# exoclime/HELIOS

Hardware: AMD Instinct MI355X
Metric: rad-conv iterations/sec x (lambda-bins x layers) (higher is better)
Workload: dtype f64; 1 GPU; BASELINE config 2: single column, 10 000 bins x 100 layers, premixed corr-k, isotropic scattering; nbin=10000, nlayer=100, ny=20, species=0, columns_per_gpu=1, columns_total=1, loop=radiative, parallelism=columns sharded, 1 per GPU

## Files before the change

### helios_amd/csrc/rt_coef_kernel.inc

```
template <int ROWS, int COEF_TPB>
__global__ void __launch_bounds__(64 * COEF_TPB) HX_COEF_KERNEL(KArgs a HX_PLANE_ARG) {
    using CT = HX_PLANE_T;
    extern __shared__ __align__(16) double smem[];
    const int col = blockIdx.y;
    if (a.done[col]) return;
    const int wave = threadIdx.x >> 6, lane = threadIdx.x & 63;
    const int ntiles = a.nblk_x * a.nparts * a.NW;
    const int TS = COEF_TPB * a.S;
    const int TSP = TS;
    const int NBX = a.coef_nbx;
    double* sh_lay = smem;
    double* sh_int = sh_lay + (size_t)a.L * TSP;
    double* sh_ray = sh_int + (size_t)a.I * TSP;
    double* sh_mu = sh_ray + (size_t)a.H * NBX;
    double* sh_dc = sh_mu + a.H;
    const size_t ncl = a.cloud_lds ? (size_t)a.H * NBX : 0;
    double* sh_g0 = sh_dc + a.H;
    double* sh_cab = sh_g0 + ncl;
    double* sh_csc = sh_cab + ncl;
    int* c_of_q = (int*)(sh_csc + ncl);
    int* x_of_q = c_of_q + TS;
    const size_t nc = (size_t)a.Y * a.X;
    const size_t wgI = nc * a.I;
    const int x_base = (blockIdx.x * COEF_TPB) / (a.NW * a.nparts) * a.nxb;
    for (int q = threadIdx.x; q < TS; q += blockDim.x) {
        const int tl = blockIdx.x * COEF_TPB + q / a.S, s_in_wave = q % a.S;
        int c = -1, xq = x_base;
        if (tl < ntiles) {
            const int wv = tl % a.NW, part = (tl / a.NW) % a.nparts, bx = tl / (a.NW * a.nparts);
            const int s_local = wv * a.S + s_in_wave;
            const int xl = s_local / a.ypb, yl = s_local - xl * a.ypb;
            const int x = bx * a.nxb + xl, y = part * a.ypb + yl;
            if (s_local < a.G && x < a.X) { c = y + a.Y * x; xq = x; }
        }
        c_of_q[q] = c;
        x_of_q[q] = xq;
    }
    {
        const double* mml = a.mmm_lay + (size_t)col * a.I;
        const double* mmi = a.mmm_int + (size_t)col * a.I;
        const double* dcu = a.dcol_u + (size_t)col * a.L;
        const double* dcl = a.dcol_l + (size_t)col * a.L;
        const double* pint = a.p_int + (size_t)col * a.I;
        const double grav = a.colpar[col].g;
        for (int h = threadIdx.x; h < a.H; h += blockDim.x) {
            if (a.iso) {
                sh_mu[h] = mml[h];
                sh_dc[h] = (pint[h] - pint[h + 1]) / grav;
            } else {
                const int i = h >> 1, ii = i + (h & 1);
                sh_mu[h] = (mmi[ii] + mml[i]) / 2.0;
                sh_dc[h] = (h & 1) ? dcu[i] : dcl[i];
            }
        }
        for (int t = threadIdx.x; t < a.H * NBX; t += blockDim.x) {
            const int xs = t / a.H, h = t - xs * a.H, x = min(x_base + xs, a.X - 1);
            const size_t src = ((size_t)col * a.X + x) * a.H + h;
            sh_ray[(size_t)h * NBX + xs] = a.half_ray[src];
            if (a.cloud_lds) {
                sh_g0[(size_t)h * NBX + xs] = a.half_g0[src];
                sh_cab[(size_t)h * NBX + xs] = a.half_cab[src];
                sh_csc[(size_t)h * NBX + xs] = a.half_csc[src];
            }
        }
    }
    __syncthreads();
    {
        const int q0 = threadIdx.x % TS, nrun = blockDim.x / TS, run = threadIdx.x / TS;
        const int cq = c_of_q[q0];
        if (a.from_table) {
            const size_t sp = nc, st = nc * a.npress;
            const double* ktable = a.coltab[col].k;
            for (int pass = 0; pass < (a.iso ? 1 : 2); pass++) {
                const int nlev = pass == 0 ? a.L : a.I;
                const TPIndex* tp = (pass == 0 ? a.tp_lay : a.tp_int) + (size_t)col * a.I;
                double* dst = pass == 0 ? sh_lay : sh_int;
                const int per = (nlev + nrun - 1) / nrun;
                const int l0 = run * per, l1 = min(nlev, l0 + per);
                int ktd = -1, ktu = -1, kpd = -1, kpu = -1;
                double c00 = 0, c01 = 0, c10 = 0, c11 = 0;
                TPIndex knext = tp[min(l0, nlev - 1)];
                for (int lev = l0; lev < l1; lev++) {
                    double v = 0.0;
                    const TPIndex k = knext;
                    knext = tp[min(lev + 1, nlev - 1)];
                    if (cq >= 0) {
                        if (k.tdown != ktd || k.tup != ktu || k.pdown != kpd || k.pup != kpu) {
                            const double* t0 = ktable + (size_t)cq + st * k.tdown;
                            const double* t1 = ktable + (size_t)cq + st * k.tup;
                            c00 = t0[sp * k.pdown];
                            c01 = t0[sp * k.pup];
                            c10 = t1[sp * k.pdown];
                            c11 = t1[sp * k.pup];
                            ktd = k.tdown; ktu = k.tup; kpd = k.pdown; kpu = k.pup;
                        }
                        v = blend_tp(c00, c01, c10, c11, k, false);
                    }
                    dst[(size_t)lev * TSP + q0] = v;
                }
            }
        } else {
            const double* opl = a.opac_wg_lay + col * wgI;
            const double* opi = a.opac_wg_int + col * wgI;
            for (int lev = run; lev < a.L; lev += nrun)
                sh_lay[(size_t)lev * TSP + q0] = cq >= 0 ? opl[(size_t)cq + nc * lev] : 0.0;
            if (!a.iso)
                for (int lev = run; lev < a.I; lev += nrun)
                    sh_int[(size_t)lev * TSP + q0] = cq >= 0 ? opi[(size_t)cq + nc * lev] : 0.0;
        }
    }
    __syncthreads();
    const int tl = blockIdx.x * COEF_TPB + wave;
    if (tl >= ntiles) return;
    const int j = lane % a.k, q = wave * a.S + lane / a.k;
    const int c = c_of_q[q], x = x_of_q[q], xs = x - x_base;
    const bool valid = c >= 0;
    const hx_rt_column cp = a.colpar[col];
    CT* ctile = HX_PLANES + col * a.coef_col + (size_t)tl * a.nplane * ROWS * 64;
    const double nmu = -cp.mu_star;
    const bool plain = a.clouds != 1 && a.scat_corr != 1 && a.g_0 == 0.0 && a.dir_beam != 1;
    const double* Fd = a.F_dir_wg + col * wgI;
    const double* Fc = a.Fc_dir_wg + col * wgI;
    auto beam_at_node = [&](int n) -> double {
        if (!(a.dir_beam == 1 && valid && n <= a.H)) return 0.0;
        if (a.iso) return Fd[(size_t)c + nc * n];
        return (n & 1) ? Fc[(size_t)c + nc * (n >> 1)] : Fd[(size_t)c + nc * (n >> 1)];
    };
    double F_here = beam_at_node(j * ROWS), F_above = beam_at_node(j * ROWS + 1);
    bool scatters = true;
    if (a.matrix) {
        bool mine = false;
#pragma unroll 1
        for (int r = 0; r < ROWS; r++) {
            const int h = j * ROWS + r;
            if (valid && h < a.H) {
                const int i = a.iso ? h : h >> 1;
                const bool lower = a.iso || (h & 1) == 0;
                const int ii = lower ? i : i + 1;
                double ray = 0.0, csc = 0.0, cab = 0.0;
                if (a.cloud_lds) {
                    cab = sh_cab[(size_t)h * NBX + xs];
                    csc = sh_csc[(size_t)h * NBX + xs];
                } else if (a.clouds == 1) {
                    const size_t src = ((size_t)col * a.X + x) * a.H + h;
                    cab = a.half_cab[src];
                    csc = a.half_csc[src];
                }
                if (a.scat == 1) ray = sh_ray[(size_t)h * NBX + xs];
                const double o_l = sh_lay[(size_t)i * TSP + q], o_i = a.iso ? o_l : sh_int[(size_t)ii * TSP + q];
                const double kap = a.iso ? o_l : (lower ? (o_i + o_l) / 2.0 : (o_l + o_i) / 2.0);
                mine = mine || single_scat_albedo(ray + csc, kap * sh_mu[h] + cab, a.w_0_limit) > a.w_0_scat_limit;
            }
        }
        const unsigned long long votes = __ballot(mine);
        const unsigned long long group = a.k >= 64 ? ~0ull : ((1ull << a.k) - 1ull) << (lane - j);
        scatters = (votes & group) != 0ull;
        if (valid && j == 0) a.trigger[col * nc + c] = scatters ? 1 : 0;
    }
    for (int r = 0; r < ROWS; r++) {
        const int h = j * ROWS + r;
        double alpha = 1.0, beta = 0.0, up = 0.0, vp = 0.0, dd = 0.0, du = 0.0;
        const double Fbot = F_here, Ftop = F_above;
        F_here = F_above;
        F_above = beam_at_node(h + 2);
        if (valid && h < a.H) {
            const int i = a.iso ? h : h >> 1;
            const bool lower = a.iso || (h & 1) == 0;
            const int ii = lower ? i : i + 1;
            double g0 = a.g_0, ray = 0.0, csc = 0.0, cab = 0.0;
            if (a.cloud_lds) {
                g0 = sh_g0[(size_t)h * NBX + xs];
                cab = sh_cab[(size_t)h * NBX + xs];
                csc = sh_csc[(size_t)h * NBX + xs];
            } else if (a.clouds == 1) {
                const size_t src = ((size_t)col * a.X + x) * a.H + h;
                g0 = a.half_g0[src];
                cab = a.half_cab[src];
                csc = a.half_csc[src];
            }
            if (a.scat == 1) ray = sh_ray[(size_t)h * NBX + xs];
            const double o_l = sh_lay[(size_t)i * TSP + q], o_i = a.iso ? o_l : sh_int[(size_t)ii * TSP + q];
            const double kap = a.iso ? o_l : (lower ? (o_i + o_l) / 2.0 : (o_l + o_i) / 2.0);
            const double mu = sh_mu[h], dcol = sh_dc[h];
            const double w0 = single_scat_albedo(ray + csc, kap * mu + cab, a.w_0_limit);
            const double dtau_gas = dcol * (kap + ray / mu);
            const double dtau = plain ? dtau_gas : dtau_gas + dcol * (cab + csc) / mu;
            const Slab s = plain ? slab_coeffs_plain(w0, dtau, a.epsi)
                                 : slab_coeffs(w0, dtau, g0, a.epsi, a.epsi2, cp.mu_star, a.scat_corr, a.i2s, a.dir_beam == 1);
            if (a.diag != nullptr && a.dir_beam == 1) {
                if (s.nlim) atomicAdd(a.diag + HX_DIAG_G_LIMITED, (unsigned long long)s.nlim);
            }
            double invM = 1.0 / s.M;
            alpha = s.P * invM;
            beta = -s.N * invM;
            double K = 2.0 * HX_PI * a.epsi * (1.0 - w0) / (s.E - w0);
            double u, v;
            if (!scatters) {
                alpha = s.trans;
                beta = 0.0;
                invM = 1.0;
                K = 2.0 * HX_PI * a.epsi;
                if (a.iso || dtau < a.dtau_limit) {
                    u = v = (1.0 - s.trans) / 2.0;
                } else {
                    const double gq = a.epsi * (s.trans - 1.0) / dtau;
                    u = 1.0 + gq;
                    v = -s.trans - gq;
                }
            } else if (a.iso || dtau < a.dtau_limit) {
                u = v = (s.N + s.M - s.P) / 2.0;
            } else {
                const double qq = (plain ? a.epsi : a.epsi / (s.E * (1.0 - w0 * g0))) * (s.P - s.M + s.N) / dtau;
                u = (s.M + s.N) + qq;
                v = -s.P - qq;
            }
            up = K * u * invM;
            vp = K * v * invM;
            if (a.dir_beam == 1 && scatters) {
                const double dn = Fbot / nmu * (s.Gm * s.M + s.Gp * s.N) - Ftop / nmu * s.Gm * s.P;
                const double upw = Ftop / nmu * (s.Gm * s.N + s.Gp * s.M) - Fbot / nmu * s.P * s.Gp;
                dd = dmin(0.0, dn) * invM;
                du = dmin(0.0, upw) * invM;
            }
            if (h == 0) {
                a.boaK[col * nc + c] = scatters ? (1.0 - w0) / (s.E - w0) : 1.0;
                a.Fdir0[col * nc + c] = a.dir_beam == 1 ? (a.F_dir_wg + col * wgI)[c] : 0.0;
            }
        }
        const size_t off = plane_off(r, lane, ROWS);
        if constexpr (sizeof(CT) == sizeof(double)) {
            __builtin_nontemporal_store(alpha, ctile + 0 * ROWS * 64 + off);
            __builtin_nontemporal_store(beta, ctile + 1 * ROWS * 64 + off);
            __builtin_nontemporal_store(up, ctile + 2 * ROWS * 64 + off);
            if (a.has_vp) __builtin_nontemporal_store(vp, ctile + (size_t)a.pl_vp * ROWS * 64 + off);
        } else {
            __builtin_nontemporal_store(plane0_code(alpha, beta), ctile + 0 * ROWS * 64 + off);
            __builtin_nontemporal_store(plane1_code(beta), ctile + 1 * ROWS * 64 + off);
            __builtin_nontemporal_store((CT)up, ctile + 2 * ROWS * 64 + off);
            if (a.has_vp) __builtin_nontemporal_store((CT)(up + vp), ctile + (size_t)a.pl_vp * ROWS * 64 + off);
        }
        if (a.dir_beam == 1) {
            __builtin_nontemporal_store((CT)dd, ctile + (size_t)a.pl_dd * ROWS * 64 + off);
            __builtin_nontemporal_store((CT)du, ctile + (size_t)(a.pl_dd + 1) * ROWS * 64 + off);
        }
    }
}
```

### helios_amd/csrc/rt_fused.h

```cpp
#pragma once
#include <string>
#include <vector>

#include "hx_common.h"

namespace hx {

struct TileGeom {
    int k, ROWS, S;
    int nxb, ypb, nparts, G, NW, threads;
    int nblk_x;
    int nblk;
    int nplane;
    int has_vp, pl_vp, pl_dd;
    size_t tile_rows;
    size_t coef_elems_per_col, flux_elems_per_col;
};

struct Species {
    double* pretab = nullptr;
    double* scat_cross = nullptr;
    double* vmr_tab = nullptr;
    bool vmr_from_tab = false;
    double weight = 0.0;
// ... 9 lines not shown
    const double *lam, *scat, *absorb;
    int nw, nr;
};

struct ProfileEntry {
    std::string name;
    hipEvent_t e0, e1;
};

}

struct hx_rt {
    hx_context* ctx;
    hx_rt_dims d;
    hx_rt_flags f;
    std::vector<hx_rt_column> cols;
    int X, Y, L, I, H, C, nsweep;
    hx::TileGeom g;
    bool have_grid = false, have_tables = false, have_planck = false, refreshed = false;
    bool keep_down = false;
    bool opac_stale = false;
    void* tp_lay = nullptr;
    void* tp_int = nullptr;
    double *T_lay_ref = nullptr, *T_int_ref = nullptr;
    int nchunk;
    int coef_tpb = 4;
    bool cloud_lds = true;
    bool serpentine = false;
    unsigned flux_launches = 0;
    double state_cache_mb = 0;
    bool generic_scans = false;
    bool conv_shmem_raised = false;
    bool coef_shmem_raised = false;

    double *interwave = nullptr, *deltawave = nullptr, *wave = nullptr, *gauss_y = nullptr,
           *gauss_w = nullptr, *ktemp = nullptr, *kpress = nullptr;
    std::vector<hx::TableSet> tables;
    std::vector<int> col_table;
    hx::TableSet* coltab = nullptr;
    hx::TableSet* coltab_ref = nullptr;
    double* planck_grid = nullptr;
    std::vector<hx::Species> species;
    void* species_dev = nullptr;
    int* abs_list = nullptr;
    int nabs = 0;
    bool species_dev_stale = true;
    double *fac_lay = nullptr, *fac_int = nullptr;
    double *spec_lay = nullptr, *spec_int = nullptr;
    double *sc_spec_lay = nullptr, *sc_spec_int = nullptr;

    hx_rt_column* colpar = nullptr;
    double *p_lay = nullptr, *p_int = nullptr, *dcol_u = nullptr, *dcol_l = nullptr;
    double *T_lay = nullptr, *T_int = nullptr;
    double *surf_albedo = nullptr, *starflux = nullptr, *Bstar = nullptr;
    double *opac_wg_lay = nullptr, *opac_wg_int = nullptr;
    double *scat_cross_lay = nullptr, *scat_cross_int = nullptr;
    double *mmm_lay = nullptr, *mmm_int = nullptr;
    double *cl_abs_lay = nullptr, *cl_abs_int = nullptr, *cl_sc_lay = nullptr, *cl_sc_int = nullptr,
           *cl_g0_lay = nullptr, *cl_g0_int = nullptr, *g0_tot_lay = nullptr, *g0_tot_int = nullptr;
    double *half_ray = nullptr, *half_g0 = nullptr, *half_cab = nullptr, *half_csc = nullptr;
    double *vmr_lay = nullptr, *vmr_int = nullptr;
    double *delta_z = nullptr, *z_lay = nullptr;
    double *dtau_u = nullptr, *dtau_l = nullptr;
    double *F_dir_wg = nullptr, *Fc_dir_wg = nullptr;
    double* F_dir_band_n = nullptr;
    double* Bn = nullptr;
// ... 49 lines not shown
```

### helios_amd/csrc/rt_fused.hip

```cpp
#include "hx_tool.h"
#include "rt_select.h"
#include "rt_species.h"

#include <algorithm>
#include <cmath>

using namespace hx;

namespace {

int rt_fail(hx_rt* rt, int code, const char* msg) { return hx_fail(rt->ctx, code, "%s", msg); }

template <class T>
int dev_alloc(hx_rt* rt, T** p, size_t n, bool zero = true) {
    void* q = nullptr;
    if (n == 0) n = 1;
    hipError_t e = hipMalloc(&q, n * sizeof(T));
    if (e != hipSuccess)
        return hx_fail(rt->ctx, -(int)e, "hipMalloc of %zu bytes failed: %s", n * sizeof(T),
                       hipGetErrorString(e));
    if (zero) {
        e = hipMemsetAsync(q, 0, n * sizeof(T), rt->ctx->stream);
        if (e != hipSuccess) return hx_fail(rt->ctx, -(int)e, "hipMemset failed");
    }
// ... 180 lines not shown
    f.keep_up = rt->matrix_keep_state ? 1 : 0;
    f.colpar = a.colpar;
    f.Bn = a.Bn; f.coef = a.coef; f.U0_in = a.U0; f.boaK = a.boaK; f.Fdir0 = a.Fdir0;
    f.surf_albedo = a.surf_albedo; f.gauss_w = a.gauss_w;
    f.Utile = a.Utile; f.Dtile = a.Dtile; f.U0 = a.U0; f.F_down_band_n = a.F_down_band_n;
    f.F_up_band_n = a.F_up_band_n;
    f.coef_col = a.coef_col; f.flux_col = a.flux_col;
    f.done = a.done;
    f.reverse = rt->serpentine ? (rt->flux_launches++ & 1) : 0;
    f.cache_state_from = INT_MAX;
    if (rt->serpentine && rt->state_cache_mb > 0) {
        const double per_wg = (double)g.nparts * g.NW * g.ROWS * 64 * sizeof(double);
        const long long total = (long long)g.nblk_x * rt->C;
        const long long keep = (long long)(rt->state_cache_mb * 1048576.0 / per_wg);
        f.cache_state_from = (int)std::max(0LL, total - keep);
    }
    if (rt->matrix) {
        f.reverse = 0;
        f.cache_state_from = INT_MAX;
    }
    (void)(rt->coef32 ? select_flux_f32(rt, &f) : select_flux<double>(rt, &f));
}

void launch_coef(hx_rt* rt, KArgs a) {
    const TileGeom& g = rt->g;
    const int ntiles = g.nblk_x * g.nparts * g.NW, tpb = rt->coef_tpb;
    a.coef_nbx = coef_nbx(rt, tpb);
    size_t shmem = coef_shmem_bytes(rt, tpb);
    const size_t cloud_image = 3 * (size_t)rt->H * a.coef_nbx * sizeof(double);
    a.cloud_lds = a.clouds == 1 && rt->cloud_lds && shmem + cloud_image <= 80 * 1024;
    if (a.cloud_lds) shmem += cloud_image;
    const dim3 grid((ntiles + tpb - 1) / tpb, rt->C);
    if (rt->coef32) select_coef_f32(rt, a, grid, shmem);
    else select_coef<double>(rt, a, grid, shmem);
}

int set_flux_shmem_limits(hx_rt* rt) {
    const size_t shmem = flux_shmem_bytes(rt);
    if (shmem > 160 * 1024) return rt_fail(rt, HX_E_UNSUPPORTED, "workgroup LDS demand exceeds 160 KiB");
    if (shmem <= 64 * 1024) return 0;
    HX_HIP(rt->ctx, rt->coef_bytes == 4 ? select_flux_f32(rt, nullptr) : select_flux<double>(rt, nullptr));
    return 0;
}

}

extern "C" {

int hx_rt_struct_sizes(int* dims_size, int* flags_size, int* column_size) {
    if (dims_size) *dims_size = (int)sizeof(hx_rt_dims);
    if (flags_size) *flags_size = (int)sizeof(hx_rt_flags);
    if (column_size) *column_size = (int)sizeof(hx_rt_column);
    return 0;
}

static int rt_create_into(hx_rt* rt, hx_context* ctx, const hx_rt_dims* dims, const hx_rt_flags* flags,
                          const hx_rt_column* columns);

int hx_rt_create(hx_context* ctx, const hx_rt_dims* dims, const hx_rt_flags* flags,
                 const hx_rt_column* columns, hx_rt** out_rt) {
    if (!ctx || !dims || !flags || !columns || !out_rt) return HX_E_ARG;
    *out_rt = nullptr;
    HX_REQUIRE(ctx, dims->nbin > 0 && dims->ny > 0 && dims->nlayer >= 1 && dims->ncol > 0, HX_E_ARG,
               "bad dimensions");
    HX_REQUIRE(ctx, dims->plancktable_dim >= 10 && dims->plancktable_step > 0, HX_E_ARG,
               "bad Planck-table dimensions");
    HX_HIP(ctx, hipSetDevice(ctx->device));
// ... 9 lines not shown

static int rt_create_into(hx_rt* rt, hx_context* ctx, const hx_rt_dims* dims, const hx_rt_flags* flags,
                          const hx_rt_column* columns) {
    rt->ctx = ctx;
    rt->d = *dims;
    rt->f = *flags;
    rt->cols.assign(columns, columns + dims->ncol);
    rt->X = dims->nbin; rt->Y = dims->ny; rt->L = dims->nlayer; rt->I = rt->L + 1;
    rt->H = flags->iso ? rt->L : 2 * rt->L;
    rt->C = dims->ncol;
    rt->have_albedo.assign(dims->ncol, 0);
    rt->col_table.assign(dims->ncol, 0);
    RT_ALLOC(rt->iter_dev, 2);
    rt->nsweep = (flags->singlewalk ? 1000 : 3) * (flags->scat ? 1 : 0) + 1;
#ifdef HX_PROFILING
    if (const char* e = getenv("HELIOS_RT_DEBUG_NSWEEP")) rt->nsweep = atoi(e);
#endif
    if (const char* e = getenv("HELIOS_RT_MATRIX"))
        return hx_fail(ctx, HX_E_ARG, "HELIOS_RT_MATRIX=%s: the knob is retired (the matrix method has one solver); unset it", e);
    rt->matrix = flags->matrix != 0;
    rt->matrix_keep_state = rt->matrix && flags->debug == 1;
    if (!choose_geometry(rt->H, rt->Y, rt->X, rt->C, flags->dir_beam, flags->scat_corr, rt->g))
        return hx_fail(ctx, HX_E_UNSUPPORTED, "fused path supports nlayer <= 1024 (2048 isothermal layers); use the per-stage API");
    rt->nchunk = std::max(1, std::min(512, std::max((rt->X + 47) / 48, std::min(32, (rt->X + 7) / 8))));
    if (const char* e = getenv("HELIOS_RT_GENERIC_SCANS")) rt->generic_scans = atoi(e) != 0;
    rt->coef_bytes = flags->coef_fp32 && !rt->matrix && coef_fp32_tiling(rt->g.ROWS, rt->g.k, rt->generic_scans) ? 4 : 8;
    if (const char* e = getenv("HELIOS_RT_CLOUD_LDS")) rt->cloud_lds = atoi(e) != 0;
    rt->coef_tpb = std::max(1, std::min(8, 16 / std::max(1, rt->g.S)));
    if (const char* e = getenv("HELIOS_RT_COEF_TPB")) rt->coef_tpb = atoi(e);
    if (rt->coef_tpb != 1 && rt->coef_tpb != 2 && !(rt->coef_tpb == 8 && rt->g.ROWS <= 16)) rt->coef_tpb = 4;
    while (rt->coef_tpb > 1 && coef_shmem_bytes(rt, rt->coef_tpb) > 150 * 1024) rt->coef_tpb /= 2;
    if (coef_shmem_bytes(rt, rt->coef_tpb) > 160 * 1024)
        return hx_fail(ctx, HX_E_UNSUPPORTED, "k_rt_coef's staging of one tile exceeds the 160 KiB of LDS");
    if (const char* e = getenv("HELIOS_RT_NCHUNK")) rt->nchunk = std::max(1, std::min(4096, atoi(e)));
    {
        const double state_mb = (double)rt->C * rt->g.flux_elems_per_col * sizeof(double) / 1048576.0;
        const double between_mb = (double)rt->C * rt->X * ((rt->H + 3) + 4.0 * rt->I) * sizeof(double) / 1048576.0;
        rt->serpentine = state_mb >= 64.0 && between_mb <= 64.0;
        rt->state_cache_mb = rt->serpentine ? 240.0 : 0.0;
    }
    if (const char* e = getenv("HELIOS_RT_SERPENTINE")) rt->serpentine = atoi(e) != 0;
    if (const char* e = getenv("HELIOS_RT_STATE_CACHE_MB")) rt->state_cache_mb = atof(e);
    rt->species.resize(dims->nspecies > 0 ? dims->nspecies : 0);
    int rc = set_flux_shmem_limits(rt);
    if (rc) return rc;

    const size_t X = rt->X, Y = rt->Y, L = rt->L, I = rt->I, C = rt->C, nc = X * Y;
    RT_ALLOC(rt->interwave, X + 1); RT_ALLOC(rt->deltawave, X); RT_ALLOC(rt->wave, X);
    RT_ALLOC(rt->gauss_y, Y); RT_ALLOC(rt->gauss_w, Y);
    RT_ALLOC(rt->ktemp, dims->ntemp); RT_ALLOC(rt->kpress, dims->npress);
    RT_ALLOC(rt->planck_grid, (size_t)(dims->plancktable_dim + 1) * X);
    RT_ALLOC(rt->colpar, C);
    RT_ALLOC(rt->coltab, C);
    RT_ALLOC(rt->coltab_ref, C);
    RT_ALLOC(rt->p_lay, C * L); RT_ALLOC(rt->p_int, C * I); RT_ALLOC(rt->dcol_u, C * L);
    RT_ALLOC(rt->dcol_l, C * L); RT_ALLOC(rt->T_lay, C * (L + 1)); RT_ALLOC(rt->T_int, C * I);
    RT_ALLOC(rt->surf_albedo, C * X); RT_ALLOC(rt->starflux, C * X); RT_ALLOC(rt->Bstar, C * X);
    RT_ALLOC(rt->opac_wg_lay, C * nc * I); RT_ALLOC(rt->opac_wg_int, C * nc * I);
    RT_ALLOC(rt->scat_cross_lay, C * X * I); RT_ALLOC(rt->scat_cross_int, C * X * I);
    RT_ALLOC(rt->mmm_lay, C * I); RT_ALLOC(rt->mmm_int, C * I);
    RT_ALLOC(rt->cl_abs_lay, C * X * I); RT_ALLOC(rt->cl_abs_int, C * X * I);
    RT_ALLOC(rt->cl_sc_lay, C * X * I); RT_ALLOC(rt->cl_sc_int, C * X * I);
    if (flags->clouds) {
        RT_ALLOC(rt->cl_g0_lay, C * X * I); RT_ALLOC(rt->cl_g0_int, C * X * I);
    }
    RT_ALLOC(rt->g0_tot_lay, C * X * I); RT_ALLOC(rt->g0_tot_int, C * X * I);
// ... 1296 lines not shown
```

### helios_amd/csrc/rt_kernels.h

```cpp
#pragma once
#include "rt_fused.h"
#include "conv_adjust.h"
#include "temp_step.h"
#include "two_stream.h"
#include "plane_code.h"

namespace hx {

struct KArgs {
    int X, Y, L, I, H, C;
    int k, ROWS, S, nxb, ypb, nparts, G, NW, nblk_x, nblk, nplane, nchunk, coef_nbx;
    int cloud_lds;
    int scat, dir_beam, clouds, scat_corr, nsweep, keep_down, real_star;
    int iso;
    int has_vp, pl_vp, pl_dd;
    int matrix;
    int* trigger;
    double Kconst;
    int dim, step;
    double epsi, epsi2, g_0, i2s, w_0_limit, w_0_scat_limit, dtau_limit;
    const hx_rt_column* colpar;
    const double *T_lay, *p_lay, *p_int, *dcol_u, *dcol_l, *surf_albedo, *Bstar, *planck_grid;
    const double *opac_wg_lay, *opac_wg_int, *scat_cross_lay, *scat_cross_int, *mmm_lay, *mmm_int;
    const double *cl_abs_lay, *cl_abs_int, *cl_sc_lay, *cl_sc_int, *g0_tot_lay, *g0_tot_int;
// ... 26 lines not shown
    double *Utile, *Dtile, *U0, *F_down_band_n, *F_up_band_n;
    size_t coef_col, flux_col;
    const int* done;
};

__device__ __forceinline__ double interface_T(const double* T, int i, int L) {
    if (i == 0) return T[0] - 0.5 * (T[1] - T[0]);
    if (i == L) return T[L - 1] + 0.5 * (T[L - 1] - T[L - 2]);
    return T[i - 1] + 0.5 * (T[i] - T[i - 1]);
}

__host__ __device__ __forceinline__ size_t plane_off(int r, int lane, int ROWS) {
    (void)ROWS;
    return (size_t)r * 64 + lane;
}

#ifndef HX_PLANE_KERNELS_ONLY
__global__ void __launch_bounds__(256) k_rt_nodes(KArgs a) {
    __shared__ double tile[32][33];
    const int col = blockIdx.z;
    if (blockIdx.x == 0 && blockIdx.y == 0 && blockIdx.z == 0 && threadIdx.x == 0 && a.iter_dev != nullptr) {
        const int cur = a.iter_dev[0];
        a.iter_dev[1] = cur;
        a.iter_dev[0] = cur + 1;
    }
    if (a.done[col]) return;
    const int NN = a.H + 3;
    const double* T = a.T_lay + (size_t)col * (a.L + 1);
    const int x0 = blockIdx.x * 32, n0 = blockIdx.y * 32;
    const int tx = threadIdx.x & 31, ty = threadIdx.x >> 5;
    if (blockIdx.x == 0 && blockIdx.y == 0)
        for (int i = threadIdx.x; i < a.I; i += blockDim.x)
            a.T_int[(size_t)col * a.I + i] = interface_T(T, i, a.L);
    for (int r = ty; r < 32; r += 8) {
        const int n = n0 + r, x = x0 + tx;
        if (n < NN && x < a.X) {
            double v;
            if (n == a.H + 1) {
                v = a.Bstar[(size_t)col * a.X + x];
            } else {
                double Tn;
                if (n == a.H + 2) Tn = T[a.L];
                else if (a.iso) Tn = T[min(n, a.L - 1)];
                else if (n & 1) Tn = T[(n - 1) >> 1];
                else Tn = interface_T(T, n >> 1, a.L);
                v = planck_lookup(a.planck_grid, Tn, x, a.X, a.dim, a.step);
            }
            tile[r][tx] = v;
        }
    }
    __syncthreads();
    for (int r = ty; r < 32; r += 8) {
        const int x = x0 + r, n = n0 + tx;
        if (n < NN && x < a.X) a.Bn[((size_t)col * a.X + x) * NN + n] = tile[tx][r];
    }
}

#endif
template <int CTRL, int ROW_MASK>
__device__ __forceinline__ double dpp_move(double v) {
    int lo = __double2loint(v), hi = __double2hiint(v);
    lo = __builtin_amdgcn_update_dpp(lo, lo, CTRL, ROW_MASK, 0xf, false);
    hi = __builtin_amdgcn_update_dpp(hi, hi, CTRL, ROW_MASK, 0xf, false);
    return __hiloint2double(hi, lo);
}

template <int N>
__device__ __forceinline__ double from_lane_below(double v, int k) {
    if (N == 1 && k == 32) return dpp_move<0x138, 0xf>(v);
    if (N < 16 && k <= 16) {
        int lo = __double2loint(v), hi = __double2hiint(v);
        lo = __builtin_amdgcn_update_dpp(lo, lo, 0x110 + (N & 15), 0xf, 0xf, false);
        hi = __builtin_amdgcn_update_dpp(hi, hi, 0x110 + (N & 15), 0xf, 0xf, false);
        return __hiloint2double(hi, lo);
    } else {
        return __shfl_up(v, N);
    }
}
template <int N>
__device__ __forceinline__ double from_lane_above(double v, int k) {
    if (N == 1 && k == 32) return dpp_move<0x130, 0xf>(v);
    if (N < 16 && k <= 16) {
// ... 207 lines not shown
                tile[q][hh][tx] = !on ? 0.0 : a.iso ? src_l[q][b_l] : (src_i[q][b_i] + src_l[q][b_l]) / 2.0;
            }
        }
    }
    __syncthreads();
    const int h = blockIdx.y * 32 + tx;
    for (int xx = ty; xx < 32; xx += 8) {
        const int xo = blockIdx.x * 32 + xx;
        if (xo < a.X && h < a.H)
            for (int q = 0; q < nq; q++) dst[q][((size_t)col * a.X + xo) * a.H + h] = tile[q][tx][xx];
    }
}

#endif

#define HX_COEF_KERNEL k_rt_coef
#define HX_PLANE_T double
#define HX_PLANE_ARG
#define HX_PLANES a.coef
#include "rt_coef_kernel.inc"
#undef HX_COEF_KERNEL
#undef HX_PLANE_T
#undef HX_PLANE_ARG
#undef HX_PLANES
#define HX_COEF_KERNEL k_rt_coef_f32
#define HX_PLANE_T float
#define HX_PLANE_ARG , float* coef32
#define HX_PLANES coef32
#include "rt_coef_kernel.inc"
#undef HX_COEF_KERNEL
#undef HX_PLANE_T
#undef HX_PLANE_ARG
#undef HX_PLANES

#ifndef HX_PLANE_KERNELS_ONLY
__global__ void __launch_bounds__(256) k_rt_dtau_halves(KArgs a) {
    const int col = blockIdx.z, i = blockIdx.y;
    const size_t nc = (size_t)a.Y * a.X;
    const size_t c = (size_t)blockIdx.x * blockDim.x + threadIdx.x;
    if (c >= nc || a.done[col]) return;
    const int x = (int)(c / a.Y);
    const size_t wgI = nc * a.I, bandI = (size_t)a.X * a.I;
    const double* opl = a.opac_wg_lay + col * wgI;
    const double* opi = a.opac_wg_int + col * wgI;
    const double* scl = a.scat_cross_lay + col * bandI;
    const double* sci = a.scat_cross_int + col * bandI;
    const double* mml = a.mmm_lay + (size_t)col * a.I;
    const double* mmi = a.mmm_int + (size_t)col * a.I;
    const size_t b = x + (size_t)a.X * i, k = c + nc * i;
    if (a.iso) {
        const double* pint = a.p_int + (size_t)col * a.I;
        const double ray = a.scat == 1 ? scl[b] : 0.0;
        a.dtau_u[col * nc * a.L + k] = (pint[i] - pint[i + 1]) / a.colpar[col].g * (opl[k] + ray / mml[i]);
        return;
    }
    double ray_up = 0, ray_low = 0;
    if (a.scat == 1) {
        ray_up = (scl[b] + sci[b + a.X]) / 2.0;
        ray_low = (sci[b] + scl[b]) / 2.0;
    }
    const double kap_up = (opl[k] + opi[k + nc]) / 2.0, kap_low = (opi[k] + opl[k]) / 2.0;
    const double mu_up = (mml[i] + mmi[i + 1]) / 2.0, mu_low = (mmi[i] + mml[i]) / 2.0;
    const size_t wgL = nc * a.L;
    a.dtau_u[col * wgL + k] = a.dcol_u[(size_t)col * a.L + i] * (kap_up + ray_up / mu_up);
    a.dtau_l[col * wgL + k] = a.dcol_l[(size_t)col * a.L + i] * (kap_low + ray_low / mu_low);
}
// ... 55 lines not shown
    }
        HX_MOEBIUS_STEP(1) HX_MOEBIUS_STEP(2) HX_MOEBIUS_STEP(4) HX_MOEBIUS_STEP(8) HX_MOEBIUS_STEP(16) HX_MOEBIUS_STEP(32)
#undef HX_MOEBIUS_STEP
    }
}

#ifndef HX_BEAM_GROUP
#define HX_BEAM_GROUP 4
#endif
#ifndef HX_BIG_ROWS_ONE_WAVE
#define HX_BIG_ROWS_ONE_WAVE 1
#endif
constexpr bool flux_one_wave(int rows) { return rows >= 15 && HX_BIG_ROWS_ONE_WAVE; }
#define HX_FLUX_HEAD __global__ void __launch_bounds__(flux_one_wave(ROWS) ? 64 : 320) k_rt_flux(FluxArgs a)
#define HX_PLANE_T double
#define HX_PLANES a.coef
#include "rt_flux_kernel.inc"
#undef HX_FLUX_HEAD
#undef HX_PLANE_T
#undef HX_PLANES
#define HX_FLUX_HEAD __device__ __forceinline__ void rt_flux_f32_body(FluxArgs a, const float* coef32)
#define HX_PLANE_T float
#define HX_PLANES coef32
#include "rt_flux_kernel.inc"
#undef HX_FLUX_HEAD
#undef HX_PLANE_T
#undef HX_PLANES
template <int ROWS, int K = 0, bool MATRIX = false>
__global__ void __launch_bounds__(flux_one_wave(ROWS) ? 64 : 320) k_rt_flux_f32(FluxArgs a, const float* coef32) {
    rt_flux_f32_body<ROWS, K, MATRIX>(a, coef32);
}

#ifndef HX_PLANE_KERNELS_ONLY
__global__ void __launch_bounds__(256) k_rt_totals_a(KArgs a) {
    const int col = blockIdx.y, chunk = blockIdx.x;
    if (a.done[col]) return;
    const int I = a.I;
    const int per = (a.X + a.nchunk - 1) / a.nchunk;
    const int x0 = chunk * per, x1 = min(a.X, x0 + per);
    const double* __restrict__ fdir = a.F_dir_band_n + (size_t)col * a.X * I;
    const double* __restrict__ dl = a.deltawave;
    for (int t = threadIdx.x; t < 2 * I; t += blockDim.x) {
        const int dir = t / I, i = t - dir * I;
        const double* __restrict__ band = (dir == 0 ? a.F_down_band_n : a.F_up_band_n) + (size_t)col * a.X * I;
        double acc = 0.0;
        for (int xb = x0; xb < x1; xb += 8) {
            double v[8];
#pragma unroll
            for (int u = 0; u < 8; u++) {
                const int x = min(xb + u, x1 - 1);
                const double f = fdir[(size_t)x * I + i], b = band[(size_t)x * I + i];
                v[u] = dir == 0 ? f + b : b;
            }
#pragma unroll
            for (int u = 0; u < 8; u++)
                if (xb + u < x1) acc += v[u] * dl[xb + u];
        }
        a.tot_part[(((size_t)col * a.nchunk + chunk) * 2) * I + t] = acc;
    }
}

struct TotalsBArgs {
    KArgs a;
    RadTempArgs rt;
    int step_temperature;
    int* done_w;
    int* iters_done;
    const int* iter_dev;
    size_t sL, sL1, sI;
};

__global__ void __launch_bounds__(1024) k_rt_totals_b(TotalsBArgs q) {
    const KArgs& a = q.a;
    const int col = blockIdx.x;
    if (a.done[col]) return;
    const int I = a.I, L = a.L;
    double* up = a.F_up_tot + (size_t)col * I;
    double* down = a.F_down_tot + (size_t)col * I;
    double* net = a.F_net + (size_t)col * I;
    __shared__ double seg[4][256];
    for (int t0 = 0; t0 < 2 * I; t0 += 256) {
        const int t = t0 + (threadIdx.x & 255), sgm = threadIdx.x >> 8;
        const int cper = (a.nchunk + 3) / 4, c0 = sgm * cper, c1 = min(a.nchunk, c0 + cper);
        double s = 0.0;
        if (t < 2 * I) {
            const double* __restrict__ part = a.tot_part + ((size_t)col * a.nchunk * 2) * I + t;
            for (int cb = c0; cb < c1; cb += 8) {
                double v[8];
#pragma unroll
// ... 378 lines not shown
```

### helios_amd/csrc/rt_select.h

```cpp
#pragma once
#include <type_traits>

#include "rt_kernels.h"

namespace hx {

template <class CT> constexpr bool planes_fp32 = std::is_same_v<CT, float>;

template <class CT> constexpr bool plane_rows(int rows) { return !planes_fp32<CT> || rows <= 14; }

template <class CT, class F>
auto for_rows(int rows, F&& fn) {
    switch (rows) {
#define HX_ROWS(n) \
    case n:        \
        if constexpr (plane_rows<CT>(n)) return fn(std::integral_constant<int, n>{}); else break;
        HX_ROWS(1) HX_ROWS(2) HX_ROWS(3) HX_ROWS(4) HX_ROWS(5) HX_ROWS(6) HX_ROWS(7) HX_ROWS(8) HX_ROWS(9) HX_ROWS(10)
        HX_ROWS(11) HX_ROWS(12) HX_ROWS(13) HX_ROWS(14) HX_ROWS(15) HX_ROWS(20) HX_ROWS(24) HX_ROWS(28) HX_ROWS(32)
#undef HX_ROWS
    }
    return fn(std::integral_constant<int, planes_fp32<CT> ? 14 : 16>{});
}

inline size_t flux_shmem_bytes(const hx_rt* rt) {
// ... 15 lines not shown
    }
    return hipSuccess;
}

template <class CT, int ROWS, bool MATRIX>
hipError_t flux_method(hx_rt* rt, const FluxArgs* f) {
    if constexpr (ROWS > 16) return flux_kernel<CT, ROWS, 64, MATRIX>(rt, f);
    else if constexpr (planes_fp32<CT> && ROWS == 14) return flux_kernel<CT, 14, 16, MATRIX>(rt, f);
    else {
        const int k = rt->generic_scans ? 0 : rt->g.k;
        if (k == 16) return flux_kernel<CT, ROWS, 16, MATRIX>(rt, f);
        if (k == 32) return flux_kernel<CT, ROWS, 32, MATRIX>(rt, f);
        if (k == 64) return flux_kernel<CT, ROWS, 64, MATRIX>(rt, f);
        return flux_kernel<CT, ROWS, 0, MATRIX>(rt, f);
    }
}

template <class CT>
hipError_t select_flux(hx_rt* rt, const FluxArgs* f) {
    return for_rows<CT>(rt->g.ROWS, [&](auto rows) {
        constexpr int ROWS = decltype(rows)::value;
        if constexpr (!planes_fp32<CT>)
            if (rt->matrix) return flux_method<CT, ROWS, true>(rt, f);
        return flux_method<CT, ROWS, false>(rt, f);
    });
}

inline int coef_nbx(const hx_rt* rt, int tpb) { return rt->g.nxb * ((tpb - 1) / (rt->g.NW * rt->g.nparts) + 2); }
inline size_t coef_shmem_bytes(const hx_rt* rt, int tpb) {
    const int TS = tpb * rt->g.S;
    return ((size_t)(rt->L + rt->I) * TS + (size_t)rt->H * (coef_nbx(rt, tpb) + 2)) * sizeof(double) + 2 * TS * sizeof(int);
}

template <class CT, int ROWS, int TPB>
void coef_kernel(hx_rt* rt, const KArgs& a, dim3 grid, size_t shmem) {
    const void* kernel;
    if constexpr (planes_fp32<CT>) kernel = (const void*)k_rt_coef_f32<ROWS, TPB>;
    else kernel = (const void*)k_rt_coef<ROWS, TPB>;
    if (shmem > 64 * 1024 && !rt->coef_shmem_raised) {
        (void)hipFuncSetAttribute(kernel, hipFuncAttributeMaxDynamicSharedMemorySize, (int)shmem);
        rt->coef_shmem_raised = true;
    }
    if constexpr (planes_fp32<CT>)
        hipLaunchKernelGGL(HIP_KERNEL_NAME(k_rt_coef_f32<ROWS, TPB>), grid, dim3(64 * TPB), shmem, rt->ctx->stream, a, rt->coef32);
    else
        hipLaunchKernelGGL(HIP_KERNEL_NAME(k_rt_coef<ROWS, TPB>), grid, dim3(64 * TPB), shmem, rt->ctx->stream, a);
}

template <class CT>
void select_coef(hx_rt* rt, const KArgs& a, dim3 grid, size_t shmem) {
    for_rows<CT>(rt->g.ROWS, [&](auto rows) {
        constexpr int ROWS = decltype(rows)::value;
        switch (rt->coef_tpb) {
            case 1: coef_kernel<CT, ROWS, 1>(rt, a, grid, shmem); break;
            case 2: coef_kernel<CT, ROWS, 2>(rt, a, grid, shmem); break;
            case 8:
                if constexpr (ROWS <= 16) { coef_kernel<CT, ROWS, 8>(rt, a, grid, shmem); break; }
                [[fallthrough]];
            default: coef_kernel<CT, ROWS, 4>(rt, a, grid, shmem); break;
        }
    });
}

bool coef_fp32_tiling(int rows, int k, bool generic_scans);
hipError_t select_flux_f32(hx_rt* rt, const FluxArgs* f);
void select_coef_f32(hx_rt* rt, const KArgs& a, dim3 grid, size_t shmem);

}
// ... 1 lines not shown
```

Measured before the change: 2.543 billion bin*layer*iterations/s.

## Specialize coef kernel for plain configs; restructure Planck tile and totals loops

Adds a compile-time specialised coefficient kernel, used when matrix, iso, direct beam, clouds and scattering correction are all off, so the runtime flag branches fold away; an env var forces the general path. Separately, the Planck tile fill is rewritten to gather temperatures and table indices for four rows at once, exposing more independent loads. The totals kernel is widened to 24-wide unrolled accumulation with 32-bit offsets and a waves-per-EU hint. This costs extra template instantiations and more register pressure in the unrolled loops. The active config (isotropic scattering, no clouds) likely fails the iso==0 check, so the plain kernel may not run.

```diff
diff --git a/helios_amd/csrc/rt_coef_kernel.inc b/helios_amd/csrc/rt_coef_kernel.inc
--- a/helios_amd/csrc/rt_coef_kernel.inc
+++ b/helios_amd/csrc/rt_coef_kernel.inc
@@ -1,4 +1,10 @@
-template <int ROWS, int COEF_TPB>
+#ifndef HX_COEF_FLAG
+#define HX_COEF_FLAG(name) a.name
+#define HX_COEF_FROM_TABLE a.from_table
+#define HX_COEF_TEMPLATE template <int ROWS, int COEF_TPB>
+#define HX_COEF_FLAG_DEFAULTS
+#endif
+HX_COEF_TEMPLATE
 __global__ void __launch_bounds__(64 * COEF_TPB) HX_COEF_KERNEL(KArgs a HX_PLANE_ARG) {
     using CT = HX_PLANE_T;
     extern __shared__ __align__(16) double smem[];
@@ -14,7 +20,7 @@
     double* sh_ray = sh_int + (size_t)a.I * TSP;
     double* sh_mu = sh_ray + (size_t)a.H * NBX;
     double* sh_dc = sh_mu + a.H;
-    const size_t ncl = a.cloud_lds ? (size_t)a.H * NBX : 0;
+    const size_t ncl = HX_COEF_FLAG(cloud_lds) ? (size_t)a.H * NBX : 0;
     double* sh_g0 = sh_dc + a.H;
     double* sh_cab = sh_g0 + ncl;
     double* sh_csc = sh_cab + ncl;
@@ -44,7 +50,7 @@
         const double* pint = a.p_int + (size_t)col * a.I;
         const double grav = a.colpar[col].g;
         for (int h = threadIdx.x; h < a.H; h += blockDim.x) {
-            if (a.iso) {
+            if (HX_COEF_FLAG(iso)) {
                 sh_mu[h] = mml[h];
                 sh_dc[h] = (pint[h] - pint[h + 1]) / grav;
             } else {
@@ -57,7 +63,7 @@
             const int xs = t / a.H, h = t - xs * a.H, x = min(x_base + xs, a.X - 1);
             const size_t src = ((size_t)col * a.X + x) * a.H + h;
             sh_ray[(size_t)h * NBX + xs] = a.half_ray[src];
-            if (a.cloud_lds) {
+            if (HX_COEF_FLAG(cloud_lds)) {
                 sh_g0[(size_t)h * NBX + xs] = a.half_g0[src];
                 sh_cab[(size_t)h * NBX + xs] = a.half_cab[src];
                 sh_csc[(size_t)h * NBX + xs] = a.half_csc[src];
@@ -68,10 +74,10 @@
     {
         const int q0 = threadIdx.x % TS, nrun = blockDim.x / TS, run = threadIdx.x / TS;
         const int cq = c_of_q[q0];
-        if (a.from_table) {
+        if (HX_COEF_FROM_TABLE) {
             const size_t sp = nc, st = nc * a.npress;
             const double* ktable = a.coltab[col].k;
-            for (int pass = 0; pass < (a.iso ? 1 : 2); pass++) {
+            for (int pass = 0; pass < (HX_COEF_FLAG(iso) ? 1 : 2); pass++) {
                 const int nlev = pass == 0 ? a.L : a.I;
                 const TPIndex* tp = (pass == 0 ? a.tp_lay : a.tp_int) + (size_t)col * a.I;
                 double* dst = pass == 0 ? sh_lay : sh_int;
@@ -104,7 +110,7 @@
             const double* opi = a.opac_wg_int + col * wgI;
             for (int lev = run; lev < a.L; lev += nrun)
                 sh_lay[(size_t)lev * TSP + q0] = cq >= 0 ? opl[(size_t)cq + nc * lev] : 0.0;
-            if (!a.iso)
+            if (!HX_COEF_FLAG(iso))
                 for (int lev = run; lev < a.I; lev += nrun)
                     sh_int[(size_t)lev * TSP + q0] = cq >= 0 ? opi[(size_t)cq + nc * lev] : 0.0;
         }
@@ -118,37 +124,37 @@
     const hx_rt_column cp = a.colpar[col];
     CT* ctile = HX_PLANES + col * a.coef_col + (size_t)tl * a.nplane * ROWS * 64;
     const double nmu = -cp.mu_star;
-    const bool plain = a.clouds != 1 && a.scat_corr != 1 && a.g_0 == 0.0 && a.dir_beam != 1;
+    const bool plain = HX_COEF_FLAG(clouds) != 1 && HX_COEF_FLAG(scat_corr) != 1 && HX_COEF_FLAG(g_0) == 0.0 && HX_COEF_FLAG(dir_beam) != 1;
     const double* Fd = a.F_dir_wg + col * wgI;
     const double* Fc = a.Fc_dir_wg + col * wgI;
     auto beam_at_node = [&](int n) -> double {
-        if (!(a.dir_beam == 1 && valid && n <= a.H)) return 0.0;
-        if (a.iso) return Fd[(size_t)c + nc * n];
+        if (!(HX_COEF_FLAG(dir_beam) == 1 && valid && n <= a.H)) return 0.0;
+        if (HX_COEF_FLAG(iso)) return Fd[(size_t)c + nc * n];
         return (n & 1) ? Fc[(size_t)c + nc * (n >> 1)] : Fd[(size_t)c + nc * (n >> 1)];
     };
     double F_here = beam_at_node(j * ROWS), F_above = beam_at_node(j * ROWS + 1);
     bool scatters = true;
-    if (a.matrix) {
+    if (HX_COEF_FLAG(matrix)) {
         bool mine = false;
 #pragma unroll 1
         for (int r = 0; r < ROWS; r++) {
             const int h = j * ROWS + r;
             if (valid && h < a.H) {
-                const int i = a.iso ? h : h >> 1;
-                const bool lower = a.iso || (h & 1) == 0;
+                const int i = HX_COEF_FLAG(iso) ? h : h >> 1;
+                const bool lower = HX_COEF_FLAG(iso) || (h & 1) == 0;
                 const int ii = lower ? i : i + 1;
                 double ray = 0.0, csc = 0.0, cab = 0.0;
-                if (a.cloud_lds) {
+                if (HX_COEF_FLAG(cloud_lds)) {
                     cab = sh_cab[(size_t)h * NBX + xs];
                     csc = sh_csc[(size_t)h * NBX + xs];
-                } else if (a.clouds == 1) {
+                } else if (HX_COEF_FLAG(clouds) == 1) {
                     const size_t src = ((size_t)col * a.X + x) * a.H + h;
                     cab = a.half_cab[src];
                     csc = a.half_csc[src];
                 }
                 if (a.scat == 1) ray = sh_ray[(size_t)h * NBX + xs];
-                const double o_l = sh_lay[(size_t)i * TSP + q], o_i = a.iso ? o_l : sh_int[(size_t)ii * TSP + q];
-                const double kap = a.iso ? o_l : (lower ? (o_i + o_l) / 2.0 : (o_l + o_i) / 2.0);
+                const double o_l = sh_lay[(size_t)i * TSP + q], o_i = HX_COEF_FLAG(iso) ? o_l : sh_int[(size_t)ii * TSP + q];
+                const double kap = HX_COEF_FLAG(iso) ? o_l : (lower ? (o_i + o_l) / 2.0 : (o_l + o_i) / 2.0);
                 mine = mine || single_scat_albedo(ray + csc, kap * sh_mu[h] + cab, a.w_0_limit) > a.w_0_scat_limit;
             }
         }
@@ -164,31 +170,31 @@
         F_here = F_above;
         F_above = beam_at_node(h + 2);
         if (valid && h < a.H) {
-            const int i = a.iso ? h : h >> 1;
-            const bool lower = a.iso || (h & 1) == 0;
+            const int i = HX_COEF_FLAG(iso) ? h : h >> 1;
+            const bool lower = HX_COEF_FLAG(iso) || (h & 1) == 0;
             const int ii = lower ? i : i + 1;
-            double g0 = a.g_0, ray = 0.0, csc = 0.0, cab = 0.0;
-            if (a.cloud_lds) {
+            double g0 = HX_COEF_FLAG(g_0), ray = 0.0, csc = 0.0, cab = 0.0;
+            if (HX_COEF_FLAG(cloud_lds)) {
                 g0 = sh_g0[(size_t)h * NBX + xs];
                 cab = sh_cab[(size_t)h * NBX + xs];
                 csc = sh_csc[(size_t)h * NBX + xs];
-            } else if (a.clouds == 1) {
+            } else if (HX_COEF_FLAG(clouds) == 1) {
                 const size_t src = ((size_t)col * a.X + x) * a.H + h;
                 g0 = a.half_g0[src];
                 cab = a.half_cab[src];
                 csc = a.half_csc[src];
             }
             if (a.scat == 1) ray = sh_ray[(size_t)h * NBX + xs];
-            const double o_l = sh_lay[(size_t)i * TSP + q], o_i = a.iso ? o_l : sh_int[(size_t)ii * TSP + q];
-            const double kap = a.iso ? o_l : (lower ? (o_i + o_l) / 2.0 : (o_l + o_i) / 2.0);
+            const double o_l = sh_lay[(size_t)i * TSP + q], o_i = HX_COEF_FLAG(iso) ? o_l : sh_int[(size_t)ii * TSP + q];
+            const double kap = HX_COEF_FLAG(iso) ? o_l : (lower ? (o_i + o_l) / 2.0 : (o_l + o_i) / 2.0);
             const double mu = sh_mu[h], dcol = sh_dc[h];
             const double w0 = single_scat_albedo(ray + csc, kap * mu + cab, a.w_0_limit);
             const double dtau_gas = dcol * (kap + ray / mu);
             const double dtau = plain ? dtau_gas : dtau_gas + dcol * (cab + csc) / mu;
             const Slab s = plain ? slab_coeffs_plain(w0, dtau, a.epsi)
-                                 : slab_coeffs(w0, dtau, g0, a.epsi, a.epsi2, cp.mu_star, a.scat_corr, a.i2s, a.dir_beam == 1);
-            if (a.diag != nullptr && a.dir_beam == 1) {
-                if (s.nlim) atomicAdd(a.diag + HX_DIAG_G_LIMITED, (unsigned long long)s.nlim);
+                                 : slab_coeffs(w0, dtau, g0, a.epsi, a.epsi2, cp.mu_star, HX_COEF_FLAG(scat_corr), a.i2s, HX_COEF_FLAG(dir_beam) == 1);
+            if (HX_COEF_FLAG(diag) != nullptr && HX_COEF_FLAG(dir_beam) == 1) {
+                if (s.nlim) atomicAdd(HX_COEF_FLAG(diag) + HX_DIAG_G_LIMITED, (unsigned long long)s.nlim);
             }
             double invM = 1.0 / s.M;
             alpha = s.P * invM;
@@ -200,14 +206,14 @@
                 beta = 0.0;
                 invM = 1.0;
                 K = 2.0 * HX_PI * a.epsi;
-                if (a.iso || dtau < a.dtau_limit) {
+                if (HX_COEF_FLAG(iso) || dtau < a.dtau_limit) {
                     u = v = (1.0 - s.trans) / 2.0;
                 } else {
                     const double gq = a.epsi * (s.trans - 1.0) / dtau;
                     u = 1.0 + gq;
                     v = -s.trans - gq;
                 }
-            } else if (a.iso || dtau < a.dtau_limit) {
+            } else if (HX_COEF_FLAG(iso) || dtau < a.dtau_limit) {
                 u = v = (s.N + s.M - s.P) / 2.0;
             } else {
                 const double qq = (plain ? a.epsi : a.epsi / (s.E * (1.0 - w0 * g0))) * (s.P - s.M + s.N) / dtau;
@@ -216,7 +222,7 @@
             }
             up = K * u * invM;
             vp = K * v * invM;
-            if (a.dir_beam == 1 && scatters) {
+            if (HX_COEF_FLAG(dir_beam) == 1 && scatters) {
                 const double dn = Fbot / nmu * (s.Gm * s.M + s.Gp * s.N) - Ftop / nmu * s.Gm * s.P;
                 const double upw = Ftop / nmu * (s.Gm * s.N + s.Gp * s.M) - Fbot / nmu * s.P * s.Gp;
                 dd = dmin(0.0, dn) * invM;
@@ -224,7 +230,7 @@
             }
             if (h == 0) {
                 a.boaK[col * nc + c] = scatters ? (1.0 - w0) / (s.E - w0) : 1.0;
-                a.Fdir0[col * nc + c] = a.dir_beam == 1 ? (a.F_dir_wg + col * wgI)[c] : 0.0;
+                a.Fdir0[col * nc + c] = HX_COEF_FLAG(dir_beam) == 1 ? (a.F_dir_wg + col * wgI)[c] : 0.0;
             }
         }
         const size_t off = plane_off(r, lane, ROWS);
@@ -232,16 +238,22 @@
             __builtin_nontemporal_store(alpha, ctile + 0 * ROWS * 64 + off);
             __builtin_nontemporal_store(beta, ctile + 1 * ROWS * 64 + off);
             __builtin_nontemporal_store(up, ctile + 2 * ROWS * 64 + off);
-            if (a.has_vp) __builtin_nontemporal_store(vp, ctile + (size_t)a.pl_vp * ROWS * 64 + off);
+            if (HX_COEF_FLAG(has_vp)) __builtin_nontemporal_store(vp, ctile + (size_t)a.pl_vp * ROWS * 64 + off);
         } else {
             __builtin_nontemporal_store(plane0_code(alpha, beta), ctile + 0 * ROWS * 64 + off);
             __builtin_nontemporal_store(plane1_code(beta), ctile + 1 * ROWS * 64 + off);
             __builtin_nontemporal_store((CT)up, ctile + 2 * ROWS * 64 + off);
-            if (a.has_vp) __builtin_nontemporal_store((CT)(up + vp), ctile + (size_t)a.pl_vp * ROWS * 64 + off);
-        }
-        if (a.dir_beam == 1) {
+            if (HX_COEF_FLAG(has_vp)) __builtin_nontemporal_store((CT)(up + vp), ctile + (size_t)a.pl_vp * ROWS * 64 + off);
+        }
+        if (HX_COEF_FLAG(dir_beam) == 1) {
             __builtin_nontemporal_store((CT)dd, ctile + (size_t)a.pl_dd * ROWS * 64 + off);
             __builtin_nontemporal_store((CT)du, ctile + (size_t)(a.pl_dd + 1) * ROWS * 64 + off);
         }
     }
 }
+#ifdef HX_COEF_FLAG_DEFAULTS
+#undef HX_COEF_FLAG
+#undef HX_COEF_FROM_TABLE
+#undef HX_COEF_TEMPLATE
+#undef HX_COEF_FLAG_DEFAULTS
+#endif
diff --git a/helios_amd/csrc/rt_fused.h b/helios_amd/csrc/rt_fused.h
--- a/helios_amd/csrc/rt_fused.h
+++ b/helios_amd/csrc/rt_fused.h
@@ -65,6 +65,8 @@
     bool generic_scans = false;
     bool conv_shmem_raised = false;
     bool coef_shmem_raised = false;
+    bool coef_general = false;
+    bool coef_plain_shmem_raised[2] = {false, false};
 
     double *interwave = nullptr, *deltawave = nullptr, *wave = nullptr, *gauss_y = nullptr,
            *gauss_w = nullptr, *ktemp = nullptr, *kpress = nullptr;
diff --git a/helios_amd/csrc/rt_fused.hip b/helios_amd/csrc/rt_fused.hip
--- a/helios_amd/csrc/rt_fused.hip
+++ b/helios_amd/csrc/rt_fused.hip
@@ -236,7 +236,10 @@
     if (a.cloud_lds) shmem += cloud_image;
     const dim3 grid((ntiles + tpb - 1) / tpb, rt->C);
     if (rt->coef32) select_coef_f32(rt, a, grid, shmem);
-    else select_coef<double>(rt, a, grid, shmem);
+    else if (coef_runs_plain(rt, a)) {
+        ProfScope ps(rt, "rt_coef_plain");
+        select_coef<double>(rt, a, grid, shmem);
+    } else select_coef<double>(rt, a, grid, shmem);
 }
 
 int set_flux_shmem_limits(hx_rt* rt) {
@@ -312,6 +315,7 @@
     while (rt->coef_tpb > 1 && coef_shmem_bytes(rt, rt->coef_tpb) > 150 * 1024) rt->coef_tpb /= 2;
     if (coef_shmem_bytes(rt, rt->coef_tpb) > 160 * 1024)
         return hx_fail(ctx, HX_E_UNSUPPORTED, "k_rt_coef's staging of one tile exceeds the 160 KiB of LDS");
+    if (const char* e = getenv("HELIOS_RT_COEF_GENERAL")) rt->coef_general = atoi(e) != 0;
     if (const char* e = getenv("HELIOS_RT_NCHUNK")) rt->nchunk = std::max(1, std::min(4096, atoi(e)));
     {
         const double state_mb = (double)rt->C * rt->g.flux_elems_per_col * sizeof(double) / 1048576.0;
diff --git a/helios_amd/csrc/rt_kernels.h b/helios_amd/csrc/rt_kernels.h
--- a/helios_amd/csrc/rt_kernels.h
+++ b/helios_amd/csrc/rt_kernels.h
@@ -82,22 +82,49 @@
     if (blockIdx.x == 0 && blockIdx.y == 0)
         for (int i = threadIdx.x; i < a.I; i += blockDim.x)
             a.T_int[(size_t)col * a.I + i] = interface_T(T, i, a.L);
-    for (int r = ty; r < 32; r += 8) {
-        const int n = n0 + r, x = x0 + tx;
-        if (n < NN && x < a.X) {
-            double v;
-            if (n == a.H + 1) {
-                v = a.Bstar[(size_t)col * a.X + x];
-            } else {
-                double Tn;
-                if (n == a.H + 2) Tn = T[a.L];
-                else if (a.iso) Tn = T[min(n, a.L - 1)];
-                else if (n & 1) Tn = T[(n - 1) >> 1];
-                else Tn = interface_T(T, n >> 1, a.L);
-                v = planck_lookup(a.planck_grid, Tn, x, a.X, a.dim, a.step);
-            }
-            tile[r][tx] = v;
-        }
+    enum { DEAD, STAR, LEVEL, INT_BOTTOM, INT_TOP, INT_MID };
+    const int x = x0 + tx, xc = min(x, a.X - 1);
+    int kind[4];
+    double Ta[4], Tb[4], star[4];
+#pragma unroll
+    for (int q = 0; q < 4; q++) {
+        const int n = n0 + ty + 8 * q, i = n >> 1;
+        int kd, ia, ib = 0;
+        if (!(n < NN && x < a.X)) { kd = DEAD; ia = 0; }
+        else if (n == a.H + 1) { kd = STAR; ia = 0; }
+        else if (n == a.H + 2) { kd = LEVEL; ia = a.L; }
+        else if (a.iso) { kd = LEVEL; ia = min(n, a.L - 1); }
+        else if (n & 1) { kd = LEVEL; ia = (n - 1) >> 1; }
+        else if (i == 0) { kd = INT_BOTTOM; ia = 0; ib = 1; }
+        else if (i == a.L) { kd = INT_TOP; ia = a.L - 1; ib = max(a.L - 2, 0); }
+        else { kd = INT_MID; ia = i - 1; ib = i; }
+        kind[q] = kd;
+        Ta[q] = T[ia];
+        Tb[q] = T[ib];
+        star[q] = kd == STAR ? a.Bstar[(size_t)col * a.X + x] : 0.0;
+    }
+    int tdown[4], tup[4];
+    double tt[4], gd[4], gu[4];
+#pragma unroll
+    for (int q = 0; q < 4; q++) {
+        double Tn = Ta[q];
+        if (kind[q] == INT_BOTTOM) Tn = Ta[q] - 0.5 * (Tb[q] - Ta[q]);
+        else if (kind[q] == INT_TOP) Tn = Ta[q] + 0.5 * (Ta[q] - Tb[q]);
+        else if (kind[q] == INT_MID) Tn = Ta[q] + 0.5 * (Tb[q] - Ta[q]);
+        double t = (Tn - 1.0) / a.step;
+        t = dmax(0.001, dmin(a.dim - 1.001, t));
+        tt[q] = t;
+        tdown[q] = (int)floor(t);
+        tup[q] = (int)ceil(t);
+        gd[q] = a.planck_grid[xc + (size_t)tdown[q] * a.X];
+        gu[q] = a.planck_grid[xc + (size_t)tup[q] * a.X];
+    }
+#pragma unroll
+    for (int q = 0; q < 4; q++) {
+        double v = gd[q];
+        if (tdown[q] != tup[q]) v = gd[q] * (tup[q] - tt[q]) + gu[q] * (tt[q] - tdown[q]);
+        if (kind[q] == STAR) v = star[q];
+        if (kind[q] != DEAD) tile[ty + 8 * q][tx] = v;
     }
     __syncthreads();
     for (int r = ty; r < 32; r += 8) {
@@ -371,6 +398,26 @@
 #undef HX_PLANE_T
 #undef HX_PLANE_ARG
 #undef HX_PLANES
+struct CoefPlainFlags {
+    static constexpr int matrix = 0, iso = 0, dir_beam = 0, clouds = 0, cloud_lds = 0, scat_corr = 0, has_vp = 0;
+    static constexpr double g_0 = 0.0;
+    static constexpr unsigned long long* diag = nullptr;
+};
+#define HX_COEF_KERNEL k_rt_coef_plain
+#define HX_PLANE_T double
+#define HX_PLANE_ARG
+#define HX_PLANES a.coef
+#define HX_COEF_FLAG(name) CoefPlainFlags::name
+#define HX_COEF_FROM_TABLE FROM_TABLE
+#define HX_COEF_TEMPLATE template <int ROWS, int COEF_TPB, bool FROM_TABLE>
+#include "rt_coef_kernel.inc"
+#undef HX_COEF_KERNEL
+#undef HX_PLANE_T
+#undef HX_PLANE_ARG
+#undef HX_PLANES
+#undef HX_COEF_FLAG
+#undef HX_COEF_FROM_TABLE
+#undef HX_COEF_TEMPLATE
 
 #ifndef HX_PLANE_KERNELS_ONLY
 __global__ void __launch_bounds__(256) k_rt_dtau_halves(KArgs a) {
@@ -492,7 +539,7 @@
 }
 
 #ifndef HX_PLANE_KERNELS_ONLY
-__global__ void __launch_bounds__(256) k_rt_totals_a(KArgs a) {
+__global__ void __launch_bounds__(256) __attribute__((amdgpu_waves_per_eu(1, 2))) k_rt_totals_a(KArgs a) {
     const int col = blockIdx.y, chunk = blockIdx.x;
     if (a.done[col]) return;
     const int I = a.I;
@@ -503,18 +550,21 @@
     for (int t = threadIdx.x; t < 2 * I; t += blockDim.x) {
         const int dir = t / I, i = t - dir * I;
         const double* __restrict__ band = (dir == 0 ? a.F_down_band_n : a.F_up_band_n) + (size_t)col * a.X * I;
+        constexpr int NB = 24;
         double acc = 0.0;
-        for (int xb = x0; xb < x1; xb += 8) {
-            double v[8];
-#pragma unroll
-            for (int u = 0; u < 8; u++) {
+        for (int xb = x0; xb < x1; xb += NB) {
+            double v[NB], w[NB];
+#pragma unroll
+            for (int u = 0; u < NB; u++) {
                 const int x = min(xb + u, x1 - 1);
-                const double f = fdir[(size_t)x * I + i], b = band[(size_t)x * I + i];
+                const unsigned o = (unsigned)x * (unsigned)I + (unsigned)i;
+                const double f = fdir[o], b = band[o];
                 v[u] = dir == 0 ? f + b : b;
+                w[u] = dl[x];
             }
 #pragma unroll
-            for (int u = 0; u < 8; u++)
-                if (xb + u < x1) acc += v[u] * dl[xb + u];
+            for (int u = 0; u < NB; u++)
+                if (xb + u < x1) acc += v[u] * w[u];
         }
         a.tot_part[(((size_t)col * a.nchunk + chunk) * 2) * I + t] = acc;
     }
diff --git a/helios_amd/csrc/rt_select.h b/helios_amd/csrc/rt_select.h
--- a/helios_amd/csrc/rt_select.h
+++ b/helios_amd/csrc/rt_select.h
@@ -71,8 +71,28 @@
     return ((size_t)(rt->L + rt->I) * TS + (size_t)rt->H * (coef_nbx(rt, tpb) + 2)) * sizeof(double) + 2 * TS * sizeof(int);
 }
 
+inline bool coef_runs_plain(const hx_rt* rt, const KArgs& a) {
+    return !rt->coef32 && !rt->coef_general && a.matrix == 0 && a.iso == 0 && a.dir_beam != 1 && a.clouds != 1 && a.cloud_lds == 0 &&
+           a.scat_corr != 1 && a.has_vp == 0 && a.g_0 == 0.0;
+}
+
+template <int ROWS, int TPB, bool FROM_TABLE>
+void coef_plain_kernel(hx_rt* rt, const KArgs& a, dim3 grid, size_t shmem) {
+    if (shmem > 64 * 1024 && !rt->coef_plain_shmem_raised[FROM_TABLE]) {
+        (void)hipFuncSetAttribute((const void*)k_rt_coef_plain<ROWS, TPB, FROM_TABLE>, hipFuncAttributeMaxDynamicSharedMemorySize, (int)shmem);
+        rt->coef_plain_shmem_raised[FROM_TABLE] = true;
+    }
+    hipLaunchKernelGGL(HIP_KERNEL_NAME(k_rt_coef_plain<ROWS, TPB, FROM_TABLE>), grid, dim3(64 * TPB), shmem, rt->ctx->stream, a);
+}
+
 template <class CT, int ROWS, int TPB>
 void coef_kernel(hx_rt* rt, const KArgs& a, dim3 grid, size_t shmem) {
+    if constexpr (!planes_fp32<CT>)
+        if (coef_runs_plain(rt, a)) {
+            if (a.from_table) coef_plain_kernel<ROWS, TPB, true>(rt, a, grid, shmem);
+            else coef_plain_kernel<ROWS, TPB, false>(rt, a, grid, shmem);
+            return;
+        }
     const void* kernel;
     if constexpr (planes_fp32<CT>) kernel = (const void*)k_rt_coef_f32<ROWS, TPB>;
     else kernel = (const void*)k_rt_coef<ROWS, TPB>;
```

Result: faster. 2.610 billion bin*layer*iterations/s, median of 6 (+2.6%).
